# Sabarna07-tech/Multimodal-RAG-for-Image-Text-Search

Measured on AMD Instinct MI355X. Metric: CLIP img-embeds/sec/GPU; kNN queries/sec on 1M×512 at top-k=10, 1/2/4/8 GPUs, higher is better.
Workload: dtype fp16 MFMA scan + f64 exact rescore; 1 GPU; BASELINE config 3 (N=1) / config 4 (N>1): brute-force cosine top-10, 1M x 512 rows per GPU, 1000-query batch; rows_per_gpu=1048576, total_rows=1048576, dim=512, top_k=10, parallelism=row-sharded x1, uncertified_queries_last_step=0, searches_in_flight=2

## Files before the change

### multimodal-rag-for-image-text-search_amd/csrc/knn.hip

```cpp
#include <algorithm>
#include <cstdlib>
#include <mutex>
#include <shared_mutex>
#include <type_traits>
#include <utility>
#include <vector>

#include "common.h"
#include "knn_generic.h"

#define AS1 __attribute__((address_space(1)))
#define AS3 __attribute__((address_space(3)))

namespace {

constexpr int TILE_ROWS = 64;
constexpr int SCAN_WAVES = 8;
constexpr int SCAN_THREADS = SCAN_WAVES * 64;
constexpr int QPW = 32;
constexpr int QPG = SCAN_WAVES * QPW;
constexpr int MAX_MERGE_ENTRIES = 4096;
constexpr int MAX_K = 256;
constexpr int MERGE_THREADS = 256;
#ifndef MRAG_SAMPLE_STRIDE
// ... 642 lines not shown
#pragma unroll
          for (int qb = 0; qb < QB; ++qb) acc[X][rb][qb][r] = ok ? acc[X][rb][qb][r] : -INFINITY;
        }
    }
    prow = tile * TILE_ROWS + 4 * g4;
    if constexpr (MODE == 2) pid = 4 * it;
    end_of_tile(true);
#ifdef MRAG_K7_STAMPS
    if constexpr (QB == 4) {
      st_sum[0] += st_mid - st0;
      st_sum[1] += st_end[0] - st_mid;
    } else {
      st_sum[1] += st_end[0] - st0;
    }
    st_sum[2] += st_end[1] - st_end[0];
    st_sum[3] += st_end[2] - st_end[1];
    st_sum[4] += 1;
#endif
  };

  if constexpr (MODE == 0) {
    if (!may_publish) {
#pragma unroll
      for (int qb = 0; qb < QB; ++qb) {
        const uint32_t t0 = __hip_atomic_load(theta_q + 16 * qb, __ATOMIC_RELAXED, __HIP_MEMORY_SCOPE_AGENT);
        if (t0 != 0) theta_f[qb] = mrag_ord2f(t0);
        thr[qb] = theta_f[qb];
      }
    }
  }
  if (my_tiles > 0) {
#pragma unroll
    for (int i = 0; i < GLDS_PER_WAVE; ++i) stage_piece(0, tile_of(0), i, lane);
    stage_labels(0, tile_of(0));
    asm volatile("s_waitcnt vmcnt(0)" ::: "memory");
    __syncthreads();
    for (int it = 0; it < my_tiles; it += 2) {
      tile_body(std::integral_constant<int, 0>{}, it);
      if (it + 1 < my_tiles) tile_body(std::integral_constant<int, 1>{}, it + 1);
    }
    if (my_tiles & 1) {
      static_for<NGROUPS>([&](auto g_c) { epi_group(g_c, std::integral_constant<int, 0>{}); });
    } else {
      static_for<NGROUPS>([&](auto g_c) { epi_group(g_c, std::integral_constant<int, 1>{}); });
    }
  }
#ifdef MRAG_K7_STAMPS
  if constexpr (MODE == 0) {
    const int wid = blockIdx.x * SCAN2_WAVES + w;
    if (lane == 0 && wid < K7_MAXWAVES)
      for (int i = 0; i < 7; ++i) g_k7_stamps[(size_t)wid * K7_NSTAMP + i] = st_sum[i];
  }
#endif

  if constexpr (MODE == 1) {
#pragma unroll
    for (int qb = 0; qb < QB; ++qb) {
      p.part_s[((size_t)split * p.Qp + slot0 + 16 * qb) * 4 + g4] = smax[qb];
    }
    return;
  }
  if constexpr (MODE == 2) {
#pragma unroll
    for (int qb = 0; qb < QB; ++qb) {
      using u32x4 = uint32_t __attribute__((ext_vector_type(4)));
      *(u32x4*)(p.rec + (((size_t)split * p.Qp + slot0 + 16 * qb) * 4 + g4) * 4) =
          u32x4{rm1[qb], rm2[qb], rm3[qb], 0u};
    }
    return;
  }
#pragma unroll
  for (int qb = 0; qb < QB; ++qb) {
    float fs[8];
    int fi[8];
#pragma unroll
    for (int j = 0; j < 8; ++j) {
      fs[j] = j < KL3 ? ls[qb][j] : -INFINITY;
      fi[j] = j < KL3 ? li[qb][j] : -1;
    }
    float tau = li[qb][KL3 - 1] >= 0 ? ls[qb][KL3 - 1] : -INFINITY;
#pragma unroll
    for (int o = 16; o < 64; o += 16) {
#pragma unroll
      for (int j = 0; j < KL3; ++j) {
        const float ps = __shfl_xor(ls[qb][j], o);
        const int pi = __shfl_xor(li[qb][j], o);
        if (pi >= 0 && ps > fs[7]) list_insert<8>(fs, fi, ps, pi);
      }
      const int plast = __shfl_xor(li[qb][KL3 - 1], o);
      const float pl = __shfl_xor(ls[qb][KL3 - 1], o);
      if (plast >= 0) tau = fmaxf(tau, pl);
    }
    if (g4 == 0) {
      const int slot = slot0 + 16 * qb;
      float* os = p.part_s + ((size_t)split * p.Qp + slot) * 8;
      int32_t* oi = p.part_i + ((size_t)split * p.Qp + slot) * 8;
#pragma unroll
      for (int j = 0; j < 8; ++j) {
        os[j] = fs[j];
        oi[j] = fi[j];
      }
      if (fi[7] >= 0) tau = fmaxf(tau, fs[7]);
      p.part_tau[(size_t)split * p.Qp + slot] = tau;
    }
  }
}

constexpr float THETA_SEED_MARGIN = (float)(2.5 * EPS_F16);
__global__ __launch_bounds__(64) void theta_init_kernel(const float* __restrict__ smax, int nvals, int Qp, int k,
                                                        uint32_t* __restrict__ theta) {
  constexpr int PER_LANE = 16;
  const int q = blockIdx.x, lane = threadIdx.x;
  float v[PER_LANE];
  const int splits = nvals / 4;
#pragma unroll
  for (int t = 0; t < 4; ++t) {
    const int sp = lane + 64 * t;
    const f32x4 x = sp < splits ? *(const f32x4*)(smax + ((size_t)sp * Qp + q) * 4)
                                : f32x4{-INFINITY, -INFINITY, -INFINITY, -INFINITY};
#pragma unroll
    for (int u = 0; u < 4; ++u) v[4 * t + u] = x[u];
  }
  float kth = -INFINITY;
  for (int r = 0; r < k; ++r) {
    float best = -INFINITY;
    int bt = 0;
#pragma unroll
    for (int t = 0; t < PER_LANE; ++t)
      if (v[t] > best) {
        best = v[t];
        bt = t;
      }
    float wbest = best;
#pragma unroll
    for (int off = 32; off > 0; off >>= 1) wbest = fmaxf(wbest, __shfl_xor(wbest, off));
    if (wbest == -INFINITY) {
      kth = -INFINITY;
      break;
    }
    const uint64_t holders = __ballot(best == wbest);
    if (lane == (int)__builtin_ctzll(holders)) {
#pragma unroll
      for (int t = 0; t < PER_LANE; ++t)
        if (t == bt) v[t] = -INFINITY;
    }
    kth = wbest;
  }
  if (lane == 0) theta[q] = (kth == -INFINITY) ? 0u : mrag_f2ord(kth - THETA_SEED_MARGIN);
}

struct ResolveParams {
  const uint32_t* rec;
  uint32_t idmask;
  int splits, Qp, k, DP, tile_step, label_filter;
  const _Float16* x16;
  const _Float16* q16;
  const int32_t* labels;
  uint32_t* theta;
  float* part_s;
  int32_t* part_i;
  float* part_tau;
};
constexpr int XLISTS = 4, XCAP = XLISTS * 8;
constexpr int REC_ID_BITS_MAX = 10;

__global__ __launch_bounds__(64) void sample_resolve_kernel(ResolveParams p) {
  using u32x4 = uint32_t __attribute__((ext_vector_type(4)));
  constexpr int PER_LANE = 32;
  __shared__ uint32_t qrec[64 * PER_LANE];
  __shared__ float xs[XCAP + 16];
  __shared__ int xr[XCAP + 16];
  const int q = blockIdx.x, lane = threadIdx.x;
  const uint64_t lt = (1ull << lane) - 1;
  uint32_t u[PER_LANE], m3 = 0u;
#pragma unroll
  for (int t = 0; t < 4; ++t) {
    const int sp = lane + 64 * t;
#pragma unroll
    for (int g = 0; g < 4; ++g) {
      const u32x4 r = sp < p.splits ? *(const u32x4*)(p.rec + (((size_t)sp * p.Qp + q) * 4 + g) * 4)
                                    : u32x4{0u, 0u, 0u, 0u};
      u[8 * t + 2 * g] = r[0];
      u[8 * t + 2 * g + 1] = r[1];
      m3 = max(m3, r[2]);
    }
  }
#pragma unroll
  for (int off = 32; off > 0; off >>= 1) m3 = max(m3, (uint32_t)__shfl_xor((int)m3, off));

  uint32_t kth = 0u, prev = ~0u;
  int above = 0;
  for (int r = 0; r < p.k; ++r) {
    uint32_t best = 0u;
    int c = 0;
#pragma unroll
    for (int i = 0; i < PER_LANE; ++i) best = max(best, u[i] < prev ? u[i] : 0u);
#pragma unroll
    for (int off = 32; off > 0; off >>= 1) best = max(best, (uint32_t)__shfl_xor((int)best, off));
    if (best <= p.idmask) break;
#pragma unroll
    for (int i = 0; i < PER_LANE; ++i) c += u[i] == best;
#pragma unroll
    for (int off = 32; off > 0; off >>= 1) c += __shfl_xor(c, off);
    above += c;
    if (above >= p.k) {
      kth = best;
      break;
    }
    prev = best;
  }
  float theta_f = -INFINITY;
  if (kth != 0u) theta_f = __uint_as_float(kth & ~p.idmask) - THETA_SEED_MARGIN;
  if (lane == 0) p.theta[q] = kth != 0u ? mrag_f2ord(theta_f) : 0u;

  int nrec = 0;
#pragma unroll
  for (int i = 0; i < PER_LANE; ++i) {
    const bool qf = u[i] > p.idmask && __uint_as_float(u[i] | p.idmask) > theta_f;
    const uint64_t b = __ballot(qf);
    if (qf)
      qrec[nrec + __popcll(b & lt)] =
          ((uint32_t)(lane + 64 * (i >> 3)) << 12) | ((uint32_t)((i >> 1) & 3) << 10) | (u[i] & p.idmask);
    nrec += __popcll(b);
  }
  __syncthreads();

  const int lab_lo = p.label_filter == MRAG_LABEL_ANY ? 0 : p.label_filter;
  const uint32_t lab_span = p.label_filter == MRAG_LABEL_ANY ? 0x7fffffffu : 0u;
  const int gsel = lane >> 4, rr = (lane >> 2) & 3, sub = lane & 3;
  const half8* qrow = (const half8*)(p.q16 + (size_t)q * p.DP);
  int cnt = 0;
  float tau_drop = -INFINITY;
  for (int base = 0; base < nrec; base += 4) {
    const bool have = base + gsel < nrec;
    const uint32_t pk = qrec[have ? base + gsel : base];
    const int sp = (int)(pk >> 12), g = (int)(pk >> 10) & 3, id = (int)(pk & p.idmask);
    const int64_t row = (int64_t)(sp + (id >> 2) * p.tile_step) * TILE_ROWS + 16 * (id & 3) + 4 * g + rr;
    const half8* xrow = (const half8*)(p.x16 + row * p.DP);
    float acc = 0.f;
    for (int c = sub; c < p.DP / 8; c += 4) {
      const half8 a = xrow[c], b = qrow[c];
#pragma unroll
      for (int e = 0; e < 8; ++e) acc += (float)a[e] * (float)b[e];
    }
    acc += __shfl_xor(acc, 1);
    acc += __shfl_xor(acc, 2);
    const int lab = p.labels[row];
    const bool take = have && sub == 0 && (uint32_t)(lab - lab_lo) <= lab_span && acc > theta_f;
    const uint64_t b = __ballot(take);
    if (take) {
      const int pos = cnt + __popcll(b & lt);
      xs[pos] = acc;
      xr[pos] = (int)row;
    }
    cnt += __popcll(b);
    __syncthreads();
    while (cnt > XCAP) {
      const float v = lane < cnt ? xs[lane] : INFINITY;
      float wmin = v;
#pragma unroll
      for (int off = 32; off > 0; off >>= 1) wmin = fminf(wmin, __shfl_xor(wmin, off));
      const int holder = (int)__builtin_ctzll(__ballot(v == wmin));
      tau_drop = fmaxf(tau_drop, wmin);
      if (lane == 0) {
        xs[holder] = xs[cnt - 1];
        xr[holder] = xr[cnt - 1];
      }
      --cnt;
      __syncthreads();
    }
  }
  if (lane < XCAP) {
    const size_t o = ((size_t)(p.splits + lane / 8) * p.Qp + q) * 8 + (lane & 7);
    p.part_s[o] = lane < cnt ? xs[lane] : -INFINITY;
    p.part_i[o] = lane < cnt ? xr[lane] : -1;
  }
  if (lane < XLISTS)
    p.part_tau[(size_t)(p.splits + lane) * p.Qp + q] =
        lane == 0 ? fmaxf(__uint_as_float(m3 | p.idmask), tau_drop) : -INFINITY;
}

using mrag_knn::exact_cosine16;

struct MergeParams {
  const float* part_s;
  const int32_t* part_i;
  int splits, KL, Qp, nq, k, M, R, Mp;
  int scan_splits;
  const float* q32;
  const double* qn;
  const float* x32;
  const double* xn;
  int D, DP;
  float* out_s;
  double* out_s64;
  int64_t* out_r;
  int64_t row_offset;
  float* thresh;
  int32_t* fail_list;
  int32_t* fail_cnt;
  int32_t* host_fail;
  const uint32_t* theta;
  const float* part_tau;
};

__device__ __forceinline__ float f32_round_down(double x) {
  float f = (float)x;
  if ((double)f > x) f = nextafterf(f, -INFINITY);
  return f;
}

template <int P>
__device__ __forceinline__ void wave_sort_keys(uint64_t (&k)[P], int lane) {
  constexpr int E = 64 * P;
#pragma unroll
  for (int size = 2; size <= E; size <<= 1) {
#pragma unroll
    for (int st = size >> 1; st > 0; st >>= 1) {
      if (st >= 64) {
        if constexpr (P == 2) {
          const uint64_t a = k[0], b = k[1];
          k[0] = a < b ? a : b;
          k[1] = a < b ? b : a;
        }
      } else {
#pragma unroll
        for (int pp = 0; pp < P; ++pp) {
          const int e = 64 * pp + lane;
          const bool asc = (e & size) == 0, lower = (lane & st) == 0;
          const uint64_t o = __shfl_xor((unsigned long long)k[pp], st);
          const uint64_t lo = k[pp] < o ? k[pp] : o, hi = k[pp] < o ? o : k[pp];
          k[pp] = (lower == asc) ? lo : hi;
        }
      }
    }
  }
}
template <int P>
__device__ __forceinline__ void wave_merge_lowest(uint64_t (&run)[P], const uint64_t (&b)[P], int lane) {
#pragma unroll
  for (int pp = 0; pp < P; ++pp) {
    const uint64_t rb = __shfl((unsigned long long)b[P - 1 - pp], 63 - lane);
    run[pp] = run[pp] < rb ? run[pp] : rb;
  }
#pragma unroll
  for (int st = 32 * P; st > 0; st >>= 1) {
    if (st >= 64) {
      if constexpr (P == 2) {
        const uint64_t a = run[0], c = run[1];
        run[0] = a < c ? a : c;
        run[1] = a < c ? c : a;
      }
    } else {
#pragma unroll
      for (int pp = 0; pp < P; ++pp) {
        const uint64_t o = __shfl_xor((unsigned long long)run[pp], st);
        const bool lower = (lane & st) == 0;
        run[pp] = lower ? (run[pp] < o ? run[pp] : o) : (run[pp] < o ? o : run[pp]);
      }
    }
  }
}

#ifdef MRAG_K7_STAMPS
constexpr int K8_NSTAMP = 8, K8_MAXBLK = 4096;
__device__ unsigned long long g_k8_stamps[K8_MAXBLK * K8_NSTAMP];
#define K8_STAMP(i) k8t[i] = __builtin_amdgcn_s_memtime()
#else
#define K8_STAMP(i)
#endif
template <int SEL>
__global__ __launch_bounds__(MERGE_THREADS) void knn_merge_kernel(MergeParams p) {
  extern __shared__ __attribute__((aligned(16))) char dsm[];
  uint64_t* keys = (uint64_t*)dsm;
  double* ex = (double*)(dsm + (size_t)p.R * 8);
  int32_t* er = (int32_t*)(dsm + (size_t)p.R * 8 + (size_t)p.Mp * 8);
  float* qs = (float*)(dsm + (size_t)p.R * 8 + (size_t)p.Mp * 12);
  float* red_f = (float*)(dsm + (size_t)p.R * 8 + (size_t)p.Mp * 12 + (size_t)p.DP * 4);
  int* red_i = (int*)(red_f + MERGE_THREADS / 64);

  const int q = blockIdx.x;
  const int tid = threadIdx.x, lane = tid & 63, wave = tid >> 6;
#ifdef MRAG_K7_STAMPS
  unsigned long long k8t[K8_NSTAMP] = {};
#endif
  K8_STAMP(0);

  float tau = -INFINITY;
  int valid = 0;
  const int ntot = p.splits * p.KL, nscan = p.scan_splits * p.KL;
  struct Raw {
    int r;
    float s;
  };
  auto load_raw = [&](int e) -> Raw {
    const int ec = e < ntot ? e : 0;
    const int sp = ec / p.KL, j = ec - sp * p.KL;
    const size_t o = ((size_t)sp * p.Qp + q) * p.KL + j;
    return Raw{p.part_i[o], p.part_s[o]};
  };
  auto make_key = [&](int e, Raw v) -> uint64_t {
    if (e >= ntot || v.r < 0) return ~0ull;
    ++valid;
    if (e % p.KL == p.KL - 1 && e < nscan) tau = fmaxf(tau, v.s);
    return ((uint64_t)(~mrag_f2ord(v.s)) << 32) | (uint32_t)v.r;
  };
  auto load_key = [&](int e) -> uint64_t { return make_key(e, load_raw(e)); };
  if (p.part_tau)
    for (int sp = tid; sp < p.splits; sp += MERGE_THREADS) tau = fmaxf(tau, p.part_tau[(size_t)sp * p.Qp + q]);
  for (int d = tid; d < p.DP; d += MERGE_THREADS) qs[d] = p.q32[(size_t)q * p.DP + d];
  if constexpr (SEL == 0) {
    for (int e = tid; e < p.R; e += MERGE_THREADS) keys[e] = load_key(e);
  } else {
    constexpr int E = 64 * SEL;
    uint64_t run[SEL];
#pragma unroll
    for (int pp = 0; pp < SEL; ++pp) run[pp] = ~0ull;
    constexpr int NW = MERGE_THREADS / 64;
    Raw nx[SEL];
#pragma unroll
    for (int pp = 0; pp < SEL; ++pp) nx[pp] = load_raw(wave * E + 64 * pp + lane);
    for (int c = wave; c * E < ntot; c += NW) {
      uint64_t ch[SEL];
#pragma unroll
      for (int pp = 0; pp < SEL; ++pp) {
        ch[pp] = make_key(c * E + 64 * pp + lane, nx[pp]);
        nx[pp] = load_raw((c + NW) * E + 64 * pp + lane);
      }
      wave_sort_keys<SEL>(ch, lane);
      wave_merge_lowest<SEL>(run, ch, lane);
    }
#pragma unroll
    for (int pp = 0; pp < SEL; ++pp) keys[wave * E + 64 * pp + lane] = run[pp];
  }
  K8_STAMP(1);
#pragma unroll
  for (int off = 32; off > 0; off >>= 1) {
    tau = fmaxf(tau, __shfl_xor(tau, off));
    valid += __shfl_xor(valid, off);
  }
  if (lane == 0) {
    red_f[wave] = tau;
    red_i[wave] = valid;
  }
  __syncthreads();
  tau = red_f[0];
  valid = red_i[0];
  for (int i = 1; i < MERGE_THREADS / 64; ++i) {
    tau = fmaxf(tau, red_f[i]);
    valid += red_i[i];
  }

  if constexpr (SEL == 0) {
    for (int size = 2; size <= p.R; size <<= 1) {
      for (int stride = size >> 1; stride > 0; stride >>= 1) {
        __syncthreads();
        for (int i = tid; i < (p.R >> 1); i += MERGE_THREADS) {
          const int lo = 2 * i - (i & (stride - 1));
          const int hi = lo + stride;
          const bool asc = (lo & size) == 0;
          const uint64_t a = keys[lo], b = keys[hi];
          if ((a > b) == asc) {
            keys[lo] = b;
            keys[hi] = a;
          }
        }
      }
    }
  } else {
    constexpr int E = 64 * SEL;
    if (wave == 0) {
      uint64_t run[SEL], other[SEL];
#pragma unroll
      for (int pp = 0; pp < SEL; ++pp) run[pp] = keys[64 * pp + lane];
      for (int w2 = 1; w2 < MERGE_THREADS / 64; ++w2) {
#pragma unroll
        for (int pp = 0; pp < SEL; ++pp) other[pp] = keys[w2 * E + 64 * pp + lane];
        wave_merge_lowest<SEL>(run, other, lane);
      }
#pragma unroll
      for (int pp = 0; pp < SEL; ++pp) keys[64 * pp + lane] = run[pp];
    }
  }
  K8_STAMP(2);
  __syncthreads();
  K8_STAMP(3);

  const int M = min(p.M, valid);
  const float a_next = (valid > M) ? mrag_ord2f(~(uint32_t)(keys[M] >> 32)) : -INFINITY;
  float th = -INFINITY;
  if (p.theta && p.theta[q] != 0u) th = mrag_ord2f(p.theta[q]);
  const double T = (double)fmaxf(fmaxf(tau, a_next), th);
  const double qn = p.qn[q];

  {
    const int grp = tid >> 4, sub = tid & 15;
    for (int m0 = 0; m0 < p.Mp; m0 += MERGE_THREADS / 16) {
      const int m = m0 + grp;
      if (m < M) {
        const int r = (int)(uint32_t)(keys[m] & 0xffffffffu);
        const double s = exact_cosine16(qs, qn, p.x32, p.xn, r, p.D, p.DP, sub);
        if (sub == 0) {
          ex[m] = s;
          er[m] = r;
        }
      } else if (sub == 0 && m < p.Mp) {
        ex[m] = -INFINITY;
        er[m] = -1;
      }
    }
  }
  K8_STAMP(4);
  if (p.Mp <= 64) {
    __syncthreads();
    if (wave == 0) {
      double sv = lane < p.Mp ? ex[lane] : -INFINITY;
      int rv = lane < p.Mp ? er[lane] : -1;
#pragma unroll
      for (int size = 2; size <= 64; size <<= 1) {
#pragma unroll
        for (int st = size >> 1; st > 0; st >>= 1) {
          const double so = __shfl_xor(sv, st);
          const int ro = __shfl_xor(rv, st);
          const bool asc = (lane & size) == 0, lower = (lane & st) == 0;
          if (mrag_before(so, ro, sv, rv) == (lower == asc)) {
            sv = so;
            rv = ro;
          }
        }
      }
      if (lane < p.Mp) {
        ex[lane] = sv;
        er[lane] = rv;
      }
    }
  }
  for (int size = 2; size <= (p.Mp <= 64 ? 1 : p.Mp); size <<= 1) {
    for (int stride = size >> 1; stride > 0; stride >>= 1) {
      __syncthreads();
      for (int i = tid; i < (p.Mp >> 1); i += MERGE_THREADS) {
        const int lo = 2 * i - (i & (stride - 1));
        const int hi = lo + stride;
        const bool asc = (lo & size) == 0;
        const double sa = ex[lo], sb = ex[hi];
        const int ra = er[lo], rb = er[hi];
        const bool b_first = mrag_before(sb, rb, sa, ra);
        if (b_first == asc) {
          ex[lo] = sb; er[lo] = rb;
          ex[hi] = sa; er[hi] = ra;
        }
      }
    }
  }
  __syncthreads();
  K8_STAMP(5);

  for (int j = tid; j < p.k; j += MERGE_THREADS) {
    const bool has = j < M;
    const double s = has ? ex[j] : -INFINITY;
    const size_t o = (size_t)q * p.k + j;
    p.out_s[o] = (float)s;
    if (p.out_s64) p.out_s64[o] = s;
    p.out_r[o] = has ? (int64_t)er[j] + p.row_offset : -1;
  }
  if (tid == 0) {
    bool cert;
    if (tau == -INFINITY && valid <= M) {
      cert = true;
    } else {
      cert = (M >= p.k) && (ex[p.k - 1] > T + EPS_F16);
    }
    if (!cert) {
      p.thresh[q] = (M >= p.k) ? f32_round_down(ex[p.k - 1] - EPS_F16) : -INFINITY;
      const int s = atomicAdd(p.fail_cnt, 1);
      p.fail_list[s] = q;
      if (p.host_fail) __hip_atomic_store(p.host_fail, 1, __ATOMIC_RELAXED, __HIP_MEMORY_SCOPE_SYSTEM);
    }
  }
#ifdef MRAG_K7_STAMPS
  K8_STAMP(6);
  if (tid == 0 && q < K8_MAXBLK)
    for (int i = 0; i < K8_NSTAMP; ++i) g_k8_stamps[(size_t)q * K8_NSTAMP + i] = k8t[i];
#endif
}

struct FinalParams {
  const int32_t* fail_list;
  const int32_t* fail_cnt;
  const int32_t* cand_cnt;
  const int32_t* cand;
  int ccap;
  double* scratch;
  const float* q32;
  const double* qn;
  const float* x32;
  const double* xn;
  int D, DP, k;
  float* out_s;
  double* out_s64;
  int64_t* out_r;
  int64_t row_offset;
  int32_t* overflow;
};

__device__ void block_select_best(double& bs, int64_t& br) {
  __shared__ double rs[MERGE_THREADS / 64];
  __shared__ int64_t rr[MERGE_THREADS / 64];
  const int lane = threadIdx.x & 63, wave = threadIdx.x >> 6;
#pragma unroll
  for (int off = 32; off > 0; off >>= 1) {
    const double os = __shfl_xor(bs, off);
    const int64_t orr = __shfl_xor(br, off);
    if (mrag_before(os, orr, bs, br)) {
      bs = os;
      br = orr;
    }
  }
  __syncthreads();
  if (lane == 0) {
    rs[wave] = bs;
    rr[wave] = br;
  }
  __syncthreads();
  bs = rs[0];
  br = rr[0];
  for (int i = 1; i < MERGE_THREADS / 64; ++i)
    if (mrag_before(rs[i], rr[i], bs, br)) {
      bs = rs[i];
      br = rr[i];
    }
}

__global__ __launch_bounds__(MERGE_THREADS) void knn_final_kernel(FinalParams p) {
  extern __shared__ __attribute__((aligned(16))) char dsm[];
  float* qs = (float*)dsm;
  const int slot = blockIdx.x;
  if (slot >= *p.fail_cnt) return;
  const int q = p.fail_list[slot];
  const int n = p.cand_cnt[slot];
  if (n > p.ccap) {
    if (threadIdx.x == 0) atomicOr(p.overflow, 1);
    return;
  }
  const int tid = threadIdx.x;
  for (int d = tid; d < p.DP; d += MERGE_THREADS) qs[d] = p.q32[(size_t)q * p.DP + d];
  __syncthreads();
  const double qn = p.qn[q];
  double* sc = p.scratch + (size_t)slot * p.ccap;
  const int32_t* cr = p.cand + (size_t)slot * p.ccap;
  for (int m = tid >> 4; m < n; m += MERGE_THREADS / 16) {
    const double s = exact_cosine16(qs, qn, p.x32, p.xn, cr[m], p.D, p.DP, tid & 15);
    if ((tid & 15) == 0) sc[m] = s;
// ... 547 lines not shown
    profile = ix->profile;
  }
  MRAG_REQUIRE(queries && out_scores && out_rows, "NULL query/output pointer");
  hipStream_t s = stream_arg ? (hipStream_t)stream_arg : ix->stream;
  const bool host = ptr_kind == MRAG_PTR_HOST;
  if (!host && !stream_arg)
    if (int rc = mrag::wait_null_stream(c->null_ev, s)) return rc;
  mrag::StreamDrain drain(s);
  const int D = ix->D, DP = ix->DP;
  const int64_t nout = nq * k;

  float* os = out_scores;
  double* os64 = out_scores64;
  int64_t* orr = out_rows;
  if (host) {
    if (int rc = ensure(c->out_s, nout * 4)) return rc;
    if (int rc = ensure(c->out_r, nout * 8)) return rc;
    os = (float*)c->out_s.p;
    orr = (int64_t*)c->out_r.p;
    if (out_scores64) {
      if (int rc = ensure(c->out_s64, nout * 8)) return rc;
      os64 = (double*)c->out_s64.p;
    }
  }
  int64_t uncertified = 0, retries = 0;
  int32_t info[8] = {0, 0, 0, 0, 0, 0, 0, 0};

  auto generic_args = [&]() {
    mrag_knn::GenericSearch ga{};
    ga.x16 = (const _Float16*)ix->x16.p;
    ga.x32 = (const float*)ix->x32.p;
    ga.xn = (const double*)ix->xn.p;
    ga.labels = (const int32_t*)ix->labels.p;
    ga.n = ix->n;
    ga.D = D;
    ga.DP = DP;
    ga.q16 = (const _Float16*)c->q16.p;
    ga.q32 = (const float*)c->q32.p;
    ga.qn = (const double*)c->qn.p;
    ga.nq = (int)nq;
    ga.k = k;
    ga.label_filter = label_filter;
    ga.row_offset = row_offset;
    ga.out_s = os;
    ga.out_s64 = os64;
    ga.out_r = orr;
    return ga;
  };

  if (ix->n == 0) {
    hipLaunchKernelGGL(fill_empty_kernel, dim3((unsigned)((nout + 255) / 256)), dim3(256), 0, s, os, os64,
                       orr, nout);
    MRAG_CHECK_LAUNCH();
  } else if (DP > 512 || k > MAX_K) {
    const float* qsrc = queries;
    if (host) {
      if (int rc = ensure(c->qin, (size_t)nq * D * 4)) return rc;
      MRAG_HIP(hipMemcpyAsync(c->qin.p, queries, (size_t)nq * D * 4, hipMemcpyHostToDevice, s));
      qsrc = (const float*)c->qin.p;
    }
    if (int rc = ensure(c->q32, (size_t)nq * DP * 4)) return rc;
    if (int rc = ensure(c->qn, (size_t)nq * 8)) return rc;
    if (int rc = ensure(c->q16, (size_t)nq * DP * 2)) return rc;
    if (int rc = launch_prep(qsrc, nq, D, DP, nq, (float*)c->q32.p, (double*)c->qn.p, (_Float16*)c->q16.p, s))
      return rc;
    if (int rc = mrag_knn::search_generic(generic_args(), c->gws, s, nullptr)) return rc;
  } else {
    const bool use_v3 = k <= 64;
    const int qb = use_v3 ? scan3_qb(nq) : 4;
    const int qpg = use_v3 ? 64 * qb : QPG;
    const int64_t qpad = use_v3 ? qpg : QPW;
    const int64_t Qp = (nq + qpad - 1) / qpad * qpad;
    const int qgroups = (int)((Qp + qpg - 1) / qpg);
    const int ntiles = (int)((ix->n + TILE_ROWS - 1) / TILE_ROWS);
    const int KL = use_v3 ? 8 : kl_for(k, DP);
    int S = std::max(1, 256 / qgroups);
    S = std::min(S, ntiles);
    S = std::min(S, MAX_MERGE_ENTRIES / KL);
    if (S >= 8) S &= ~7;
    const int min_tiles = ntiles / S;
    const int stride = sample_stride_for(k);
    const bool sampled = use_v3 && qb == 4 && min_tiles >= 4 * stride;
    const int max_sample_tiles = ((ntiles + S - 1) / S + stride - 1) / stride;
    int idbits = 2;
    while ((1 << idbits) < 4 * max_sample_tiles) ++idbits;
    const bool counting = sampled && counting_sample_for(k) && idbits <= REC_ID_BITS_MAX;
    const int SX = counting ? XLISTS : 0;
    const int M = std::min<int>(k + 32, S * KL);
    const int R = (int)next_pow2((int64_t)(S + SX) * KL);
    const int Mp = (int)next_pow2(std::max(M, 2));
    info[0] = S;
    info[1] = (int32_t)Qp;
    info[7] = KL;

    const float* qsrc = queries;
    if (host) {
      if (int rc = ensure(c->qin, (size_t)nq * D * 4)) return rc;
      MRAG_HIP(hipMemcpyAsync(c->qin.p, queries, (size_t)nq * D * 4, hipMemcpyHostToDevice, s));
      qsrc = (const float*)c->qin.p;
    }
    if (int rc = ensure(c->q32, (size_t)Qp * DP * 4)) return rc;
    if (int rc = ensure(c->qn, (size_t)Qp * 8)) return rc;
    if (int rc = ensure(c->q16, (size_t)Qp * DP * 2)) return rc;
    if (int rc = ensure(c->part_s, (size_t)(S + SX) * Qp * KL * 4)) return rc;
    if (int rc = ensure(c->part_i, (size_t)(S + SX) * Qp * KL * 4)) return rc;
    if (int rc = ensure(c->thresh, (size_t)Qp * 4)) return rc;
    if (int rc = ensure(c->fail_list, (size_t)Qp * 4)) return rc;
    if (int rc = ensure(c->counters, 16)) return rc;
    if (int rc = ensure(c->cand_cnt, (size_t)Qp * 4)) return rc;
    if (int rc = ensure(c->theta, (size_t)Qp * 4)) return rc;
    if (use_v3)
      if (int rc = ensure(c->part_tau, (size_t)(S + SX) * Qp * 4)) return rc;
    if (counting)
      if (int rc = ensure(c->rec, (size_t)S * Qp * 16 * 4)) return rc;

    if (int rc = launch_prep(qsrc, nq, D, DP, Qp, (float*)c->q32.p, (double*)c->qn.p, (_Float16*)c->q16.p, s,
                             PrepClear{(int32_t*)c->counters.p, (int32_t*)c->cand_cnt.p, (uint32_t*)c->theta.p}))
      return rc;

    ScanParams sp{};
    sp.theta = (uint32_t*)c->theta.p;

    sp.x16 = (const _Float16*)ix->x16.p;
    sp.labels = (const int32_t*)ix->labels.p;
    sp.q16 = (const _Float16*)c->q16.p;
    sp.ntiles = ntiles;
    sp.qgroups = qgroups;
    sp.splits = S;
    sp.Qp = (int)Qp;
    sp.label_filter = label_filter;
    sp.part_s = (float*)c->part_s.p;
    sp.part_i = (int32_t*)c->part_i.p;
    sp.fail_list = (const int32_t*)c->fail_list.p;
    sp.fail_cnt = (const int32_t*)c->counters.p;
    sp.thresh = (const float*)c->thresh.p;
    sp.cand_cnt = (int32_t*)c->cand_cnt.p;
    sp.k = k;
    sp.part_tau = use_v3 ? (float*)c->part_tau.p : nullptr;

    const scan_fn scan = use_v3 ? get_scan3(DP, 0, qb) : get_scan(DP, KL, false);
    const scan_fn collect = get_scan(DP, 8, true);
    if (!scan || !collect) return mrag::fail(MRAG_ERR_UNSUPPORTED, "no scan kernel for DP=%d", DP);
    const dim3 sgrid((unsigned)(qgroups * S));
    sp.sample_stride = stride;
    if (sampled) {
      sp.sample_tiles = min_tiles / stride;
      if (counting) {
        sp.rec = (uint32_t*)c->rec.p;
        sp.rec_keep = ~((1u << idbits) - 1u);
      }
      hipLaunchKernelGGL(get_scan3(DP, counting ? 2 : 1, qb), sgrid, dim3(SCAN2_THREADS), 0, s, sp);
      MRAG_CHECK_LAUNCH();
      if (counting) {
        ResolveParams rp{};
        rp.rec = sp.rec;
        rp.idmask = ~sp.rec_keep;
        rp.splits = S;
        rp.Qp = (int)Qp;
        rp.k = k;
        rp.DP = DP;
        rp.tile_step = S * stride;
        rp.label_filter = label_filter;
        rp.x16 = sp.x16;
        rp.q16 = sp.q16;
        rp.labels = sp.labels;
        rp.theta = sp.theta;
        rp.part_s = sp.part_s;
        rp.part_i = sp.part_i;
        rp.part_tau = sp.part_tau;
        hipLaunchKernelGGL(sample_resolve_kernel, dim3((unsigned)nq), dim3(64), 0, s, rp);
        sp.skip_magic = (uint32_t)((1ull << 32) / (uint64_t)(stride - 1) + 1);
      } else {
        hipLaunchKernelGGL(theta_init_kernel, dim3((unsigned)nq), dim3(64), 0, s, (const float*)sp.part_s, 4 * S,
                           (int)Qp, k, sp.theta);
      }
      MRAG_CHECK_LAUNCH();
    }
    if (profile) MRAG_HIP(hipEventRecord(c->ev0, s));
    hipLaunchKernelGGL(scan, sgrid, dim3(use_v3 ? SCAN2_THREADS : SCAN_THREADS), 0, s, sp);
    MRAG_CHECK_LAUNCH();
    if (profile) MRAG_HIP(hipEventRecord(c->ev1, s));

    MergeParams mp{};
    mp.part_s = sp.part_s;
    mp.part_i = sp.part_i;
    mp.splits = S + SX;
    mp.scan_splits = S;
    mp.KL = KL;
    mp.Qp = (int)Qp;
    mp.nq = (int)nq;
    mp.k = k;
    mp.M = M;
    mp.R = R;
    mp.Mp = Mp;
    mp.q32 = (const float*)c->q32.p;
    mp.qn = (const double*)c->qn.p;
    mp.x32 = (const float*)ix->x32.p;
    mp.xn = (const double*)ix->xn.p;
    mp.D = D;
    mp.DP = DP;
    mp.out_s = os;
    mp.out_s64 = os64;
    mp.out_r = orr;
    mp.row_offset = row_offset;
    mp.thresh = (float*)c->thresh.p;
    mp.fail_list = (int32_t*)c->fail_list.p;
    mp.fail_cnt = (int32_t*)c->counters.p;
    mp.theta = (const uint32_t*)c->theta.p;
    mp.part_tau = sp.part_tau;
    mp.host_fail = c->host_fail;
    __atomic_store_n(c->host_fail, 0, __ATOMIC_RELAXED);
    const int sel = M + 1 <= 64 ? 1 : (M + 1 <= 128 ? 2 : 0);
    mp.R = sel ? std::max(R, 4 * 64 * sel) : R;
    const size_t msh = (size_t)mp.R * 8 + (size_t)Mp * 12 + (size_t)DP * 4 + 64;
    auto merge = sel == 1 ? knn_merge_kernel<1> : sel == 2 ? knn_merge_kernel<2> : knn_merge_kernel<0>;
    hipLaunchKernelGGL(merge, dim3((unsigned)nq), dim3(MERGE_THREADS), msh, s, mp);
    MRAG_CHECK_LAUNCH();

    if (int rc = wait_stream(c, s)) return rc;
    if (__atomic_load_n(c->host_fail, __ATOMIC_ACQUIRE)) {
      MRAG_HIP(hipMemcpyAsync(c->host_counters, c->counters.p, 8, hipMemcpyDeviceToHost, s));
      if (int rc = wait_stream(c, s)) return rc;
    } else {
      c->host_counters[0] = 0;
    }
    if (profile) {
      float ms = 0.f;
      MRAG_HIP(hipEventElapsedTime(&ms, c->ev0, c->ev1));
      std::lock_guard<std::mutex> lk(ix->pool_mu);
      ix->scan_ms += ms;
      ix->scan_launches++;
    }
    uncertified = c->host_counters[0];
    if (uncertified > 0) {
      const int ccap = (int)std::max<int64_t>(256, std::min<int64_t>(4096, ((int64_t)64 << 20) / Qp));
      if (int rc = ensure(c->cand, (size_t)Qp * ccap * 4)) return rc;
      if (int rc = ensure(c->scratch, (size_t)Qp * ccap * 8)) return rc;
      sp.cand = (int32_t*)c->cand.p;
      sp.ccap = ccap;
      const int cgroups = (int)((uncertified + QPG - 1) / QPG);
      int Sc = std::max(S, 1024 / cgroups);
      Sc = std::min(Sc, ntiles);
      if (Sc >= 8) Sc &= ~7;
      sp.qgroups = cgroups;
      sp.splits = Sc;
      info[2] = cgroups;
      info[3] = Sc;
      info[4] = ccap;
      info[5] = (int32_t)uncertified;
      hipLaunchKernelGGL(collect, dim3((unsigned)(cgroups * Sc)), dim3(SCAN_THREADS), 0, s, sp);
      MRAG_CHECK_LAUNCH();
      FinalParams fp{};
      fp.fail_list = sp.fail_list;
      fp.fail_cnt = sp.fail_cnt;
      fp.cand_cnt = sp.cand_cnt;
      fp.cand = sp.cand;
      fp.ccap = ccap;
      fp.scratch = (double*)c->scratch.p;
      fp.q32 = mp.q32;
      fp.qn = mp.qn;
      fp.x32 = mp.x32;
      fp.xn = mp.xn;
      fp.D = D;
      fp.DP = DP;
      fp.k = k;
      fp.out_s = os;
      fp.out_s64 = os64;
      fp.out_r = orr;
      fp.row_offset = row_offset;
      fp.overflow = (int32_t*)c->counters.p + 1;
      hipLaunchKernelGGL(knn_final_kernel, dim3((unsigned)uncertified), dim3(MERGE_THREADS), (size_t)DP * 4, s, fp);
      MRAG_CHECK_LAUNCH();
      MRAG_HIP(hipMemcpyAsync(c->host_counters, c->counters.p, 8, hipMemcpyDeviceToHost, s));
      if (int rc = wait_stream(c, s)) return rc;
      info[6] = c->host_counters[1];
      if (c->host_counters[1] != 0) {
        retries = 1;
        if (int rc = mrag_knn::search_generic(generic_args(), c->gws, s, nullptr)) return rc;
      }
    }
  }

  if (host) {
    MRAG_HIP(hipMemcpyAsync(out_scores, os, nout * 4, hipMemcpyDeviceToHost, s));
    MRAG_HIP(hipMemcpyAsync(out_rows, orr, nout * 8, hipMemcpyDeviceToHost, s));
    if (out_scores64) MRAG_HIP(hipMemcpyAsync(out_scores64, os64, nout * 8, hipMemcpyDeviceToHost, s));
  }
  if (int rc = wait_stream(c, s)) return rc;
  drain.armed = false;
  std::lock_guard<std::mutex> lk(ix->pool_mu);
  ix->last_uncertified = uncertified;
  ix->last_retries = retries;
  ix->last_ctx = c;
  std::copy(info, info + 8, ix->last_info);
  return MRAG_OK;
}

#ifdef MRAG_K7_STAMPS
__attribute__((visibility("default"))) int mrag_debug_knn_last_collect(mrag_knn_index* ix, int32_t* info,
                                                                       int32_t* fail_list, int32_t* cand_cnt,
                                                                       float* thresh, int64_t nthresh) {
  MRAG_REQUIRE(ix != nullptr && info != nullptr, "NULL argument");
  std::lock_guard<std::mutex> lk(ix->pool_mu);
  std::copy(ix->last_info, ix->last_info + 8, info);
  SearchCtx* c = ix->last_ctx;
  if (!c) return MRAG_OK;
  mrag::DeviceGuard g(ix->device);
  const int64_t unc = ix->last_info[5];
  MRAG_HIP(hipDeviceSynchronize());
  if (fail_list && unc > 0) MRAG_HIP(hipMemcpy(fail_list, c->fail_list.p, unc * 4, hipMemcpyDeviceToHost));
  if (cand_cnt && unc > 0) MRAG_HIP(hipMemcpy(cand_cnt, c->cand_cnt.p, unc * 4, hipMemcpyDeviceToHost));
  if (thresh && nthresh > 0 && (size_t)nthresh * 4 <= c->thresh.bytes)
    MRAG_HIP(hipMemcpy(thresh, c->thresh.p, nthresh * 4, hipMemcpyDeviceToHost));
  return MRAG_OK;
}
#endif

int mrag_topk_merge(const double* scores64, const int64_t* rows, int32_t nlists, int64_t nq, int32_t k,
                    float* out_scores, double* out_scores64, int64_t* out_rows, void* stream) {
  MRAG_REQUIRE(nlists >= 1 && nq >= 0 && k >= 1 && k <= mrag_knn::GENERIC_MAX_K, "bad shape nlists=%d nq=%lld k=%d", nlists,
               (long long)nq, k);
  if (nq == 0) return MRAG_OK;
  MRAG_REQUIRE(scores64 && rows && out_scores && out_rows, "NULL pointer");
// ... 9 lines not shown
```

Before: 1.082 million queries/s (1000-query batches, each query scanned against a 1M x 512 shard per GPU, top-10; aggregate over GPUs).

## Widen sample resolve kernel to 256 threads and prune exact rescore candidates

The sample resolve kernel grows from one wave to four waves per query. It is templated on DP so the row dot products can be fully unrolled with the query vector staged in LDS, uses DPP-based wave reductions, and computes cross-wave prefix counts for candidate insertion. Separately, the merge kernel binary-searches the sorted fp16 scores and only exact-rescores candidates whose score lies within a 2*EPS_F16 bound of the k-th. That cuts the f64 rescoring work, but the bound has to be correct, otherwise exactness suffers. The resolve changes add extra block syncs per step, and the kernel now exists only for DP values 128, 256, 384 and 512.

Result: no change. 1.088 million queries/s (1000-query batches, each query scanned against a 1M x 512 shard per GPU, top-10; aggregate over GPUs), median of 6 (+0.5%).

```diff
diff --git a/multimodal-rag-for-image-text-search_amd/csrc/knn.hip b/multimodal-rag-for-image-text-search_amd/csrc/knn.hip
--- a/multimodal-rag-for-image-text-search_amd/csrc/knn.hip
+++ b/multimodal-rag-for-image-text-search_amd/csrc/knn.hip
@@ -818,7 +818,7 @@
 struct ResolveParams {
   const uint32_t* rec;
   uint32_t idmask;
-  int splits, Qp, k, DP, tile_step, label_filter;
+  int splits, Qp, k, tile_step, label_filter;
   const _Float16* x16;
   const _Float16* q16;
   const int32_t* labels;
@@ -829,121 +829,193 @@
 };
 constexpr int XLISTS = 4, XCAP = XLISTS * 8;
 constexpr int REC_ID_BITS_MAX = 10;
-
-__global__ __launch_bounds__(64) void sample_resolve_kernel(ResolveParams p) {
+constexpr int RESOLVE_THREADS = 256;
+constexpr int RESOLVE_STEP_GROUPS = RESOLVE_THREADS / 16;
+
+template <int CTRL>
+__device__ __forceinline__ uint32_t dpp_u32(uint32_t v) {
+  return (uint32_t)__builtin_amdgcn_update_dpp(0, (int)v, CTRL, 0xf, 0xf, true);
+}
+__device__ __forceinline__ uint32_t wave_max_u32(uint32_t v) {
+  v = max(v, dpp_u32<0xB1>(v));
+  v = max(v, dpp_u32<0x4E>(v));
+  v = max(v, dpp_u32<0x141>(v));
+  v = max(v, dpp_u32<0x140>(v));
+  const uint32_t a = (uint32_t)__builtin_amdgcn_readlane((int)v, 0), b = (uint32_t)__builtin_amdgcn_readlane((int)v, 16);
+  const uint32_t c = (uint32_t)__builtin_amdgcn_readlane((int)v, 32), d = (uint32_t)__builtin_amdgcn_readlane((int)v, 48);
+  return max(max(a, b), max(c, d));
+}
+__device__ __forceinline__ uint32_t wave_sum_u32(uint32_t v) {
+  v += dpp_u32<0xB1>(v);
+  v += dpp_u32<0x4E>(v);
+  v += dpp_u32<0x141>(v);
+  v += dpp_u32<0x140>(v);
+  return (uint32_t)__builtin_amdgcn_readlane((int)v, 0) + (uint32_t)__builtin_amdgcn_readlane((int)v, 16) +
+         (uint32_t)__builtin_amdgcn_readlane((int)v, 32) + (uint32_t)__builtin_amdgcn_readlane((int)v, 48);
+}
+
+template <int DP>
+__global__ __launch_bounds__(RESOLVE_THREADS, 4) void sample_resolve_kernel(ResolveParams p) {
   using u32x4 = uint32_t __attribute__((ext_vector_type(4)));
   constexpr int PER_LANE = 32;
+  constexpr int NCH = DP / 32;
+  constexpr int STEP_ROWS = 4 * RESOLVE_STEP_GROUPS;
   __shared__ uint32_t qrec[64 * PER_LANE];
-  __shared__ float xs[XCAP + 16];
-  __shared__ int xr[XCAP + 16];
-  const int q = blockIdx.x, lane = threadIdx.x;
+  __shared__ float xs[XCAP + STEP_ROWS];
+  __shared__ int xr[XCAP + STEP_ROWS];
+  __shared__ int wcnt[RESOLVE_THREADS / 64];
+  __shared__ half8 qs[DP / 8];
+  __shared__ int sh_nrec;
+  __shared__ float sh_theta;
+  const int q = blockIdx.x, tid = threadIdx.x, lane = tid & 63, wave = tid >> 6;
   const uint64_t lt = (1ull << lane) - 1;
-  uint32_t u[PER_LANE], m3 = 0u;
-#pragma unroll
-  for (int t = 0; t < 4; ++t) {
-    const int sp = lane + 64 * t;
-#pragma unroll
-    for (int g = 0; g < 4; ++g) {
-      const u32x4 r = sp < p.splits ? *(const u32x4*)(p.rec + (((size_t)sp * p.Qp + q) * 4 + g) * 4)
-                                    : u32x4{0u, 0u, 0u, 0u};
-      u[8 * t + 2 * g] = r[0];
-      u[8 * t + 2 * g + 1] = r[1];
-      m3 = max(m3, r[2]);
-    }
-  }
-#pragma unroll
-  for (int off = 32; off > 0; off >>= 1) m3 = max(m3, (uint32_t)__shfl_xor((int)m3, off));
-
-  uint32_t kth = 0u, prev = ~0u;
-  int above = 0;
-  for (int r = 0; r < p.k; ++r) {
-    uint32_t best = 0u;
-    int c = 0;
-#pragma unroll
-    for (int i = 0; i < PER_LANE; ++i) best = max(best, u[i] < prev ? u[i] : 0u);
-#pragma unroll
-    for (int off = 32; off > 0; off >>= 1) best = max(best, (uint32_t)__shfl_xor((int)best, off));
-    if (best <= p.idmask) break;
-#pragma unroll
-    for (int i = 0; i < PER_LANE; ++i) c += u[i] == best;
-#pragma unroll
-    for (int off = 32; off > 0; off >>= 1) c += __shfl_xor(c, off);
-    above += c;
-    if (above >= p.k) {
-      kth = best;
-      break;
-    }
-    prev = best;
-  }
-  float theta_f = -INFINITY;
-  if (kth != 0u) theta_f = __uint_as_float(kth & ~p.idmask) - THETA_SEED_MARGIN;
-  if (lane == 0) p.theta[q] = kth != 0u ? mrag_f2ord(theta_f) : 0u;
-
-  int nrec = 0;
-#pragma unroll
-  for (int i = 0; i < PER_LANE; ++i) {
-    const bool qf = u[i] > p.idmask && __uint_as_float(u[i] | p.idmask) > theta_f;
-    const uint64_t b = __ballot(qf);
-    if (qf)
-      qrec[nrec + __popcll(b & lt)] =
-          ((uint32_t)(lane + 64 * (i >> 3)) << 12) | ((uint32_t)((i >> 1) & 3) << 10) | (u[i] & p.idmask);
-    nrec += __popcll(b);
+  const int rr = (lane >> 2) & 3, sub = lane & 3;
+
+  if (tid >= RESOLVE_THREADS - DP / 8)
+    qs[tid - (RESOLVE_THREADS - DP / 8)] = ((const half8*)(p.q16 + (size_t)q * DP))[tid - (RESOLVE_THREADS - DP / 8)];
+
+  uint32_t m3 = 0u;
+  if (wave == 0) {
+    uint32_t u[PER_LANE];
+#pragma unroll
+    for (int t = 0; t < 4; ++t) {
+      const int sp = lane + 64 * t;
+#pragma unroll
+      for (int g = 0; g < 4; ++g) {
+        const u32x4 r = sp < p.splits ? *(const u32x4*)(p.rec + (((size_t)sp * p.Qp + q) * 4 + g) * 4)
+                                      : u32x4{0u, 0u, 0u, 0u};
+        u[8 * t + 2 * g] = r[0];
+        u[8 * t + 2 * g + 1] = r[1];
+        m3 = max(m3, r[2]);
+      }
+    }
+    m3 = wave_max_u32(m3);
+
+    uint32_t kth = 0u, prev = ~0u;
+    int above = 0;
+    for (int r = 0; r < p.k; ++r) {
+      uint32_t best = 0u, c = 0u;
+#pragma unroll
+      for (int i = 0; i < PER_LANE; ++i) best = max(best, u[i] < prev ? u[i] : 0u);
+      best = wave_max_u32(best);
+      if (best <= p.idmask) break;
+#pragma unroll
+      for (int i = 0; i < PER_LANE; ++i) c += u[i] == best;
+      above += (int)wave_sum_u32(c);
+      if (above >= p.k) {
+        kth = best;
+        break;
+      }
+      prev = best;
+    }
+    float theta_f = -INFINITY;
+    if (kth != 0u) theta_f = __uint_as_float(kth & ~p.idmask) - THETA_SEED_MARGIN;
+
+    int nrec = 0;
+#pragma unroll
+    for (int i = 0; i < PER_LANE; ++i) {
+      const bool qf = u[i] > p.idmask && __uint_as_float(u[i] | p.idmask) > theta_f;
+      const uint64_t b = __ballot(qf);
+      if (qf)
+        qrec[nrec + __popcll(b & lt)] =
+            ((uint32_t)(lane + 64 * (i >> 3)) << 12) | ((uint32_t)((i >> 1) & 3) << 10) | (u[i] & p.idmask);
+      nrec += __popcll(b);
+    }
+    if (lane == 0) {
+      p.theta[q] = kth != 0u ? mrag_f2ord(theta_f) : 0u;
+      sh_nrec = nrec;
+      sh_theta = theta_f;
+    }
   }
   __syncthreads();
+  const int nrec = sh_nrec;
+  const float theta_f = sh_theta;
 
   const int lab_lo = p.label_filter == MRAG_LABEL_ANY ? 0 : p.label_filter;
   const uint32_t lab_span = p.label_filter == MRAG_LABEL_ANY ? 0x7fffffffu : 0u;
-  const int gsel = lane >> 4, rr = (lane >> 2) & 3, sub = lane & 3;
-  const half8* qrow = (const half8*)(p.q16 + (size_t)q * p.DP);
   int cnt = 0;
   float tau_drop = -INFINITY;
-  for (int base = 0; base < nrec; base += 4) {
-    const bool have = base + gsel < nrec;
-    const uint32_t pk = qrec[have ? base + gsel : base];
-    const int sp = (int)(pk >> 12), g = (int)(pk >> 10) & 3, id = (int)(pk & p.idmask);
-    const int64_t row = (int64_t)(sp + (id >> 2) * p.tile_step) * TILE_ROWS + 16 * (id & 3) + 4 * g + rr;
-    const half8* xrow = (const half8*)(p.x16 + row * p.DP);
+  for (int base = 0; base < nrec; base += RESOLVE_STEP_GROUPS) {
+    const int gi = base + (tid >> 4);
+    const bool have = gi < nrec;
     float acc = 0.f;
-    for (int c = sub; c < p.DP / 8; c += 4) {
-      const half8 a = xrow[c], b = qrow[c];
-#pragma unroll
-      for (int e = 0; e < 8; ++e) acc += (float)a[e] * (float)b[e];
+    int lab = 0;
+    int64_t row = 0;
+    if (have) {
+      const uint32_t pk = qrec[gi];
+      const int sp = (int)(pk >> 12), g = (int)(pk >> 10) & 3, id = (int)(pk & p.idmask);
+      row = (int64_t)(sp + (id >> 2) * p.tile_step) * TILE_ROWS + 16 * (id & 3) + 4 * g + rr;
+      const half8* xrow = (const half8*)(p.x16 + row * DP);
+      half8 xv[NCH];
+#pragma unroll
+      for (int j = 0; j < NCH; ++j) xv[j] = xrow[sub + 4 * j];
+      lab = p.labels[row];
+      {
+#pragma clang fp contract(off)
+#pragma unroll
+        for (int j = 0; j < NCH; ++j) {
+          const half8 qc = qs[sub + 4 * j];
+#pragma unroll
+          for (int e = 0; e < 8; ++e) acc += (float)xv[j][e] * (float)qc[e];
+        }
+      }
     }
     acc += __shfl_xor(acc, 1);
     acc += __shfl_xor(acc, 2);
-    const int lab = p.labels[row];
     const bool take = have && sub == 0 && (uint32_t)(lab - lab_lo) <= lab_span && acc > theta_f;
     const uint64_t b = __ballot(take);
+    if (lane == 0) wcnt[wave] = __popcll(b);
+    __syncthreads();
+    int pos = cnt + __popcll(b & lt), tot = 0;
+#pragma unroll
+    for (int w = 0; w < RESOLVE_THREADS / 64; ++w) {
+      const int c = wcnt[w];
+      pos += w < wave ? c : 0;
+      tot += c;
+    }
     if (take) {
-      const int pos = cnt + __popcll(b & lt);
       xs[pos] = acc;
       xr[pos] = (int)row;
     }
-    cnt += __popcll(b);
+    cnt += tot;
     __syncthreads();
     while (cnt > XCAP) {
-      const float v = lane < cnt ? xs[lane] : INFINITY;
-      float wmin = v;
-#pragma unroll
-      for (int off = 32; off > 0; off >>= 1) wmin = fminf(wmin, __shfl_xor(wmin, off));
-      const int holder = (int)__builtin_ctzll(__ballot(v == wmin));
-      tau_drop = fmaxf(tau_drop, wmin);
-      if (lane == 0) {
-        xs[holder] = xs[cnt - 1];
-        xr[holder] = xr[cnt - 1];
+      if (wave == 0) {
+        const float v0 = lane < cnt ? xs[lane] : INFINITY, v1 = lane + 64 < cnt ? xs[lane + 64] : INFINITY;
+        float wmin = fminf(v0, v1);
+#pragma unroll
+        for (int off = 32; off > 0; off >>= 1) wmin = fminf(wmin, __shfl_xor(wmin, off));
+        const uint64_t b0 = __ballot(v0 == wmin), b1 = __ballot(v1 == wmin);
+        const int holder = b0 ? (int)__builtin_ctzll(b0) : 64 + (int)__builtin_ctzll(b1);
+        tau_drop = fmaxf(tau_drop, wmin);
+        if (lane == 0) {
+          xs[holder] = xs[cnt - 1];
+          xr[holder] = xr[cnt - 1];
+        }
       }
       --cnt;
       __syncthreads();
     }
   }
-  if (lane < XCAP) {
-    const size_t o = ((size_t)(p.splits + lane / 8) * p.Qp + q) * 8 + (lane & 7);
-    p.part_s[o] = lane < cnt ? xs[lane] : -INFINITY;
-    p.part_i[o] = lane < cnt ? xr[lane] : -1;
-  }
-  if (lane < XLISTS)
-    p.part_tau[(size_t)(p.splits + lane) * p.Qp + q] =
-        lane == 0 ? fmaxf(__uint_as_float(m3 | p.idmask), tau_drop) : -INFINITY;
+  if (tid < XCAP) {
+    const size_t o = ((size_t)(p.splits + tid / 8) * p.Qp + q) * 8 + (tid & 7);
+    p.part_s[o] = tid < cnt ? xs[tid] : -INFINITY;
+    p.part_i[o] = tid < cnt ? xr[tid] : -1;
+  }
+  if (tid < XLISTS)
+    p.part_tau[(size_t)(p.splits + tid) * p.Qp + q] =
+        tid == 0 ? fmaxf(__uint_as_float(m3 | p.idmask), tau_drop) : -INFINITY;
+}
+
+using resolve_fn = void (*)(ResolveParams);
+resolve_fn get_resolve(int DP) {
+  switch (DP) {
+    case 128: return sample_resolve_kernel<128>;
+    case 256: return sample_resolve_kernel<256>;
+    case 384: return sample_resolve_kernel<384>;
+    case 512: return sample_resolve_kernel<512>;
+    default: return nullptr;
+  }
 }
 
 using mrag_knn::exact_cosine16;
@@ -1159,11 +1231,23 @@
   const double T = (double)fmaxf(fmaxf(tau, a_next), th);
   const double qn = p.qn[q];
 
+  int Mq = M;
+  if (M > p.k) {
+    const double bound = (double)mrag_ord2f(~(uint32_t)(keys[p.k - 1] >> 32)) - 2.0 * EPS_F16;
+    int lo = p.k, hi = M;
+    while (lo < hi) {
+      const int mid = (lo + hi) >> 1;
+      if ((double)mrag_ord2f(~(uint32_t)(keys[mid] >> 32)) >= bound) lo = mid + 1;
+      else hi = mid;
+    }
+    Mq = lo;
+  }
+
   {
     const int grp = tid >> 4, sub = tid & 15;
     for (int m0 = 0; m0 < p.Mp; m0 += MERGE_THREADS / 16) {
       const int m = m0 + grp;
-      if (m < M) {
+      if (m < Mq) {
         const int r = (int)(uint32_t)(keys[m] & 0xffffffffu);
         const double s = exact_cosine16(qs, qn, p.x32, p.xn, r, p.D, p.DP, sub);
         if (sub == 0) {
@@ -2017,13 +2101,14 @@
       hipLaunchKernelGGL(get_scan3(DP, counting ? 2 : 1, qb), sgrid, dim3(SCAN2_THREADS), 0, s, sp);
       MRAG_CHECK_LAUNCH();
       if (counting) {
+        const resolve_fn resolve = get_resolve(DP);
+        if (!resolve) return mrag::fail(MRAG_ERR_UNSUPPORTED, "no resolve kernel for DP=%d", DP);
         ResolveParams rp{};
         rp.rec = sp.rec;
         rp.idmask = ~sp.rec_keep;
         rp.splits = S;
         rp.Qp = (int)Qp;
         rp.k = k;
-        rp.DP = DP;
         rp.tile_step = S * stride;
         rp.label_filter = label_filter;
         rp.x16 = sp.x16;
@@ -2033,7 +2118,7 @@
         rp.part_s = sp.part_s;
         rp.part_i = sp.part_i;
         rp.part_tau = sp.part_tau;
-        hipLaunchKernelGGL(sample_resolve_kernel, dim3((unsigned)nq), dim3(64), 0, s, rp);
+        hipLaunchKernelGGL(resolve, dim3((unsigned)nq), dim3(RESOLVE_THREADS), 0, s, rp);
         sp.skip_magic = (uint32_t)((1ull << 32) / (uint64_t)(stride - 1) + 1);
       } else {
         hipLaunchKernelGGL(theta_init_kernel, dim3((unsigned)nq), dim3(64), 0, s, (const float*)sp.part_s, 4 * S,
```
